# mschauer/ZigZagBoomerang.jl

Hardware: AMD Instinct MI355X
Metric: reflection events/sec, d=16384 local ZigZag (spdmp), ensemble of independent chains (higher is better)
Workload: dtype f64

## Files before the change

zigzagboomerang.jl_amd/csrc/pdmp_engine.hpp:

```cpp
#pragma once
#include <cstdint>
#include <string>
#include <vector>

#include "../../include/pdmp_mi355.h"
#ifdef PDMP_EXTRA_KERNELS
#include "../../include/pdmp_debug.h"
#endif

namespace pdmp {

struct alignas(64) ZzRec {
    double x;
    double th;
    double t;
    double I;
    double t_old;
    double a, b;
    uint64_t acc;
};
static_assert(sizeof(ZzRec) == 64, "record must be one 64-byte sector");

struct alignas(128) TrRec {
    double x, th, tx, I;
    double g, gd, tg;
    uint64_t acc;
    double a, b, t_old, tprop;
    double gb, gdb, tacc, pad;
};
static_assert(sizeof(TrRec) == 128, "tracked record must be one 128-byte line");
struct alignas(128) TrRecP {
    double x, th, tx, I;
    double g, gd, tg;
    uint64_t acc;
    double c, c100, gam0, gam1;
    double gam2, gam3, tacc, gam4;
};
static_assert(sizeof(TrRecP) == 128 && offsetof(TrRecP, tacc) == offsetof(TrRec, tacc), "same line, same tacc slot");

struct alignas(128) TrLine {
    double key0, told0, key1, told1;
    double th0, g0, gd0, tg0;
    double th1, g1, gd1, tg1;
    double c0, c100_0, c1, c100_1;
};
static_assert(sizeof(TrLine) == 128, "one line per coordinate pair");
struct alignas(32) TrCold {
    double x, tx, I;
    uint64_t acc;
};
static_assert(sizeof(TrCold) == 32, "one sector per coordinate");

struct alignas(128) DevChain {
    pdmp_chain_counters c;
    uint64_t seed;
    double t0;
    double t_event;
    double tl_scale;
    uint64_t pad[3];
};
static_assert(sizeof(DevChain) == 128, "chain header is 128 bytes");

#if defined(__HIPCC__)
__device__ __forceinline__ DevChain devchain_fresh(uint64_t seed, double t0, uint64_t ntrace, uint64_t nevents, uint64_t ndraw_main) {
    DevChain h;
    h.c.t_last = t0;
    h.c.num = 0;
    h.c.nacc = 0;
    h.c.nrefresh = 0;
    h.c.ntrace = ntrace;
    h.c.nevents = nevents;
    h.c.ndraw_main = ndraw_main;
    h.c.ndraw_global = 0;
    h.c.status = PDMP_CHAIN_OK;
    h.c.reserved = 0;
    h.seed = seed;
    h.t0 = t0;
    h.t_event = t0;
    h.tl_scale = 0.0;
    for (int k = 0; k < 3; ++k) h.pad[k] = 0;
    return h;
}

constexpr uint32_t PDMP_PRIO_TURN = 256u;
struct PrioTurn {
    uint32_t slot, it;
    __device__ __forceinline__ PrioTurn() : slot((uint32_t)__builtin_amdgcn_s_getreg(4 | (0 << 6) | (3 << 11)) & 3u), it(0) {}
    __device__ __forceinline__ void step() {
        if ((it & (PDMP_PRIO_TURN - 1u)) == 0u) {
            const uint32_t pr = ((it / PDMP_PRIO_TURN) + slot) & 3u;
            switch (pr) {
                case 0: __builtin_amdgcn_s_setprio(0); break;
                case 1: __builtin_amdgcn_s_setprio(1); break;
                case 2: __builtin_amdgcn_s_setprio(2); break;
                default: __builtin_amdgcn_s_setprio(3); break;
            }
        }
        it += 1;
    }
};

#ifndef PDMP_PRIO_LAG_K
#define PDMP_PRIO_LAG_K 32u
#endif
constexpr uint32_t PDMP_PRIO_BOARD_ROWS = 1u << 15, PDMP_PRIO_BOARD_SLOTS = 16u;
constexpr uint32_t PDMP_PRIO_BOARD_WORDS = PDMP_PRIO_BOARD_ROWS * PDMP_PRIO_BOARD_SLOTS;
struct PrioLag {
    PrioTurn turn;
    uint32_t* row;
    uint32_t slot, tag, it;
    double t_begin, scale;
    __device__ __forceinline__ PrioLag(uint32_t* board, uint32_t epoch, double t_begin_, double T) : row(nullptr), slot(0), tag(epoch << 24), it(0), t_begin(t_begin_), scale(0.0) {
        const double span = T - t_begin_;
        if (board != nullptr && epoch != 0u && span > 0.0 && span < __builtin_inf()) {
            const uint32_t xcc = (uint32_t)__builtin_amdgcn_s_getreg(20 | (0 << 6) | (3 << 11));
            const uint32_t hw = (uint32_t)__builtin_amdgcn_s_getreg(4 | (4 << 6) | (11 << 11));
            slot = (uint32_t)__builtin_amdgcn_s_getreg(4 | (0 << 6) | (3 << 11)) & (PDMP_PRIO_BOARD_SLOTS - 1u);
            row = board + (size_t)(((xcc << 12) | hw) & (PDMP_PRIO_BOARD_ROWS - 1u)) * PDMP_PRIO_BOARD_SLOTS;
            scale = 16777216.0 / span;
        }
    }
    __device__ __forceinline__ void step(double t_last, int lane) {
        if (row == nullptr) {
            turn.step();
            return;
        }
        if ((it & (PDMP_PRIO_LAG_K - 1u)) == 0u) {
            const double f = (t_last - t_begin) * scale;
            const uint32_t q = (f > 0.0) ? ((f < 16777214.0) ? (uint32_t)f : 0xfffffeu) : 0u;
            if (lane == 0) __hip_atomic_store(row + slot, tag | q, __ATOMIC_RELAXED, __HIP_MEMORY_SCOPE_AGENT);
            uint32_t w = 0u;
            if (lane < (int)PDMP_PRIO_BOARD_SLOTS) w = __hip_atomic_load(row + lane, __ATOMIC_RELAXED, __HIP_MEMORY_SCOPE_AGENT);
            const uint32_t wq = w & 0xffffffu;
            const bool behind = lane < (int)PDMP_PRIO_BOARD_SLOTS && (w & 0xff000000u) == tag && wq != 0xffffffu && (wq < q || (wq == q && (uint32_t)lane < slot));
            const uint32_t rank = (uint32_t)__popcll(__ballot(behind));
            switch (rank) {
                case 0: __builtin_amdgcn_s_setprio(3); break;
                case 1: __builtin_amdgcn_s_setprio(2); break;
                case 2: __builtin_amdgcn_s_setprio(1); break;
                default: __builtin_amdgcn_s_setprio(0); break;
            }
        }
        it += 1;
    }
    __device__ __forceinline__ void finish(int lane) {
        if (row != nullptr && lane == 0) __hip_atomic_store(row + slot, tag | 0xffffffu, __ATOMIC_RELAXED, __HIP_MEMORY_SCOPE_AGENT);
    }
};
#endif

struct CoordConst {
    double c, c100;
    uint32_t cp, k;
    double gam[5];
};
static_assert(sizeof(CoordConst) == 64, "half a line");

struct BarrierEntry {
    double lo, hi;
    double klo, khi;
    uint32_t rules;
    uint32_t pad;
};
static_assert(sizeof(BarrierEntry) == 40, "barrier table entry");
constexpr uint64_t BARRIER_ACT_HIT = 0, BARRIER_ACT_REFLECT = 1, BARRIER_ACT_UNFREEZE = 2;

struct ZzTables {
    const uint32_t* __restrict__ colptr;
    const uint32_t* __restrict__ rowval;
    const double* __restrict__ bval;
    const double* __restrict__ tval;
    const double* __restrict__ gmu_b;
    const double* __restrict__ gmu_t;
    const uint32_t* __restrict__ sptr;
    const uint32_t* __restrict__ sidx;
    const uint32_t* __restrict__ qptr;
    const uint8_t* __restrict__ pos;
    const uint8_t* __restrict__ selfpos;
    const double* __restrict__ c_shared;
    const double2* __restrict__ c2_shared;
    const CoordConst* __restrict__ cc_shared;
    const double* __restrict__ sigma;
    const double* __restrict__ gam8;
    const uint16_t* __restrict__ nb16;
};

constexpr uint32_t PDMP_LAUNCH_COUNT_LIMIT = 0xC0000000u;

struct ZzRunParams {
    ZzTables tb;
    ZzRec* rec;
    double* keys;
    DevChain* hdr;
    pdmp_event* ev;
    double* c_chain;
    double* dbg;
    int64_t dbg_cap;
    const uint64_t* __restrict__ blob;
    const uint32_t* __restrict__ tix;
    uint32_t blob_w, blob_w_pad, blob_sw, blob_pw, blob_kmax;
    uint32_t common_tix;
    int64_t d;
    int64_t dk;
    int64_t trace_cap;
    uint32_t nblk;
    uint32_t nblk_pad;
    double T;
    double factor;
    double lambda_ref;
    int32_t flags;
    int32_t adapt;
    int32_t has_refresh;
    int32_t move_all;
    int32_t force_spec4;
    int32_t track_two_sums;
    int32_t track_mean;
    uint32_t count_limit;
    uint32_t typ_extra;
    double hw_gain, hw_ahead;
    uint32_t hw_target;
    int32_t n_cu;
    int32_t helper_wave;
    uint32_t* prio_board;
    uint32_t prio_epoch;
    void* tl_lines;
    void* tl_cold;
    int32_t lattice_n;
    uint32_t lattice_magic;
    const uint64_t* __restrict__ g8_line;
// ... 368 lines not shown
```

zigzagboomerang.jl_amd/csrc/pdmp_trackp.hip:

```cpp
#include <hip/hip_runtime.h>

#include <cstdint>

#include "../../include/pdmp_detmath.h"
#include "pdmp_device.hpp"
#include "pdmp_engine.hpp"

namespace pdmp {

namespace {

__device__ __forceinline__ uint32_t w_grp8_min_u32(uint32_t v) {
    uint32_t o = (uint32_t)__builtin_amdgcn_mov_dpp((int)v, 0xB1, 0xf, 0xf, true);
    v = (o < v) ? o : v;
    o = (uint32_t)__builtin_amdgcn_mov_dpp((int)v, 0x4E, 0xf, 0xf, true);
    v = (o < v) ? o : v;
    o = (uint32_t)__builtin_amdgcn_mov_dpp((int)v, 0x141, 0xf, 0xf, true);
    return (o < v) ? o : v;
}
__device__ __forceinline__ uint32_t p_enc(double key, double tb, uint32_t pos) {
    double dlt = key - tb;
    dlt = (dlt > 0.0) ? dlt : 0.0;
    const uint32_t b = __float_as_uint((float)dlt);
    return (((b >= 8u) ? b - 8u : 0u) & ~7u) | pos;
}
__device__ __forceinline__ uint32_t p_thr(double tau, double tb) {
    double dlt = tau - tb;
    dlt = (dlt > 0.0) ? dlt : 0.0;
    return __float_as_uint((float)dlt) + 1u;
}
__device__ __forceinline__ double p_dec(uint32_t bits, double tb) {
    return pdmp_below(tb + (double)__uint_as_float(bits & ~7u));
}
constexpr uint32_t P_INFBITS = 0x7f7ffff8u;
__device__ __forceinline__ uint32_t lbf_pos(const unsigned char* smem, uint32_t b) {
    return reinterpret_cast<const uint32_t*>(smem)[b] & 7u;
}

}

template <bool HW, bool BIG = false>
struct WL {
    static_assert(!(HW && BIG), "the two-wave form keeps 2048 block bounds");
    static constexpr uint32_t NBLK = BIG ? 8192 : 2048;
    static constexpr uint32_t XO = (NBLK - 2048) * 4;
    static constexpr uint32_t LB = 0;
    static constexpr uint32_t EX = XO + 8192;
    static constexpr uint32_t URING = XO + 8704;
    static constexpr uint32_t SLB = XO + (HW ? 9792 : 9728);
    static constexpr uint32_t TB = XO + (HW ? 9920 : 9856);
    static constexpr uint32_t ACL = XO + (HW ? 10048 : 9984);
    static constexpr uint32_t NB = XO + (HW ? 10144 : 10016);
    static constexpr uint32_t CTL = 10272;
    static constexpr uint32_t HPF = 10336;
    static constexpr uint32_t RING = 10464;
    static constexpr int CMAX = HW ? 64 : 56;
    static constexpr uint32_t WIN = HW ? 256u : 128u;
    static constexpr uint32_t BYTES = HW ? RING + 512 * 16 : NB + 128;
};
constexpr uint32_t W_NR = 512;
constexpr uint32_t W_BYTES_1W = WL<false>::BYTES, W_BYTES_BIG = WL<false, true>::BYTES;
constexpr uint32_t W_BYTES_HW = WL<true>::BYTES;
constexpr int W_AMAX = 8;
#ifndef W_GROW
#define W_GROW 1.02
#define W_SHRINK 0.98
#define W_SLACK 5u
#endif
#ifndef W_HEAD_ONE_PASS
#define W_HEAD_ONE_PASS 1
#endif
#define W_TARGET_HW 48u
#define W_GAIN_HW 0.3
#define W_TARGET_1W 44u
#define W_TARGET_1W_MAX_PER_CU 12
#define W_NHYP 8
#define W_NHYP_1W 4
#define W_PF_AHEAD 1.0
static_assert(WL<false>::BYTES <= 10240, "16 chains per CU: 160 KB / 16");
static_assert(WL<false>::URING + WL<false>::WIN * 8 <= WL<false>::SLB && WL<false, true>::URING + WL<false, true>::WIN * 8 <= WL<false, true>::SLB &&
                  WL<false>::ACL + W_AMAX * 2 <= WL<false>::NB,
              "the one-wave forms' ring of draws ends where the event blocks begin");
static_assert(WL<false, true>::BYTES <= 40960, "d <= 65536: 4 chains per CU (one per SIMD), 160 KB / 4");
static_assert(W_BYTES_HW == WL<true>::RING + W_NR * 16 && W_BYTES_HW <= 20480, "8 chains per CU: 160 KB / 8");
struct WCtl {
    uint32_t filled;
    uint32_t consumed;
    uint32_t exitf;
    uint32_t pad;
    double pf_tau, pf_dt, pf_tb;
};
typedef volatile __attribute__((address_space(3))) WCtl* WCtlPtr;
__device__ __forceinline__ WCtlPtr w_ctl(unsigned char* smem, uint32_t offset) {
    return (WCtlPtr)(__attribute__((address_space(3))) unsigned char*)(smem + offset);
}

namespace {
__device__ __forceinline__ bool nb_has(const uint4 nb, uint32_t v2) {
    const uint32_t x0 = nb.x ^ v2, x1 = nb.y ^ v2, x2 = nb.z ^ v2, x3 = nb.w ^ v2;
    const uint32_t z = ((x0 - 0x00010001u) & ~x0) | ((x1 - 0x00010001u) & ~x1) | ((x2 - 0x00010001u) & ~x2) | ((x3 - 0x00010001u) & ~x3);
    return (z & 0x80008000u) != 0u;
}
__device__ __forceinline__ uint32_t nb_count(const uint4 nb) {
    const uint64_t hi = ((uint64_t)nb.w << 32) | nb.z, lo = ((uint64_t)nb.y << 32) | nb.x;
    const uint32_t ph = (~hi == 0ull) ? 4u : ((uint32_t)__builtin_clzll(~hi) >> 4);
    const uint32_t pl = (~lo == 0ull) ? 4u : ((uint32_t)__builtin_clzll(~lo) >> 4);
    return 8u - ((ph == 4u) ? 4u + pl : ph);
}
}

template <bool LAT>
__device__ __forceinline__ void trackp_helper(const ZzRunParams& P, unsigned char* smem, const int lane, const int64_t chain, const uint64_t seed,
                                           const uint64_t nm0) {
    using L = WL<true, false>;
    const WCtlPtr ctl = w_ctl(smem, L::CTL);
    double2* const ring = reinterpret_cast<double2*>(smem + L::RING);
    const uint4* const lb4 = reinterpret_cast<const uint4*>(smem + L::LB);
    const int64_t d = P.d;
    const char* const recb = reinterpret_cast<const char*>(reinterpret_cast<const TrRecP*>(P.rec) + chain * d);
    const char* const kpb = reinterpret_cast<const char*>(reinterpret_cast<const double2*>(P.keys) + chain * P.dk);
    uint16_t* const HPF = reinterpret_cast<uint16_t*>(smem + L::HPF);
    uint32_t filled = 0, sink = 0;
    double pf_done = -PDMP_INF;
    for (;;) {
        if (ctl->exitf != 0u) break;
        bool did = false;
        const uint32_t cons = ctl->consumed;
        while (filled + 64u <= cons + W_NR) {
            const uint32_t n = filled + (uint32_t)lane;
            const double u = pdmp_u01(seed, PDMP_STREAM_MAIN, nm0 + (uint64_t)n);
            ring[n & (W_NR - 1u)] = make_double2(u, pdmp_log(u));
            PDMP_LDS_ORDER();
            filled += 64u;
            if (lane == 0) ctl->filled = filled;
            did = true;
        }
        const double tau = ctl->pf_tau, dts = ctl->pf_dt, tbs = ctl->pf_tb;
        const double target = tau + P.hw_ahead * dts;
        if (target > pf_done) {
            const uint32_t lo = (pf_done > tbs) ? p_thr(pf_done, tbs) : 0u;
            const uint32_t hi0 = p_thr(target, tbs), hi = (hi0 < P_INFBITS) ? hi0 : P_INFBITS - 1u;
            uint32_t cm = 0;
#pragma unroll
            for (int j = 7; j >= 0; --j) {
                const uint4 v = lb4[lane + 64 * j];
                cm = (cm << 4) | ((v.x > lo && v.x <= hi) ? 1u : 0u) | ((v.y > lo && v.y <= hi) ? 2u : 0u) | ((v.z > lo && v.z <= hi) ? 4u : 0u) |
                     ((v.w > lo && v.w <= hi) ? 8u : 0u);
            }
            const uint32_t ncl = (uint32_t)__builtin_popcount(cm);
            const uint32_t incl = scan_add_u32(ncl);
            const uint32_t tot = (uint32_t)__builtin_amdgcn_readlane((int)incl, 63);
            uint32_t ix = incl - ncl, m_ = cm;
            while (m_ != 0u) {
                const uint32_t j = (uint32_t)(__ffs((int)m_) - 1);
// ... 98 lines not shown
                const uint32_t k = 8u * (uint32_t)s + (uint32_t)j;
                const bool in = 8u * k + (uint32_t)g < nblk;
                const double v = kp[(in ? (size_t)64 * k : (size_t)0) + (size_t)lane].x;
                vn[j] = in ? v : PDMP_INF;
            }
        };
        load8(0);
#pragma unroll
        for (int s = 0; s < 32; ++s) {
            double vc[8];
#pragma unroll
            for (int j = 0; j < 8; ++j) vc[j] = vn[j];
            __builtin_amdgcn_sched_barrier(0);
            if (s + 1 < 32) load8(s + 1);
            __builtin_amdgcn_sched_barrier(0);
            double keep = PDMP_INF;
            uint32_t kpos = 0u;
#pragma unroll
            for (int j = 0; j < 8; ++j) {
                const double v = vc[j];
                const double m = grp8_min_f64(v);
                const uint32_t pos = w_grp8_min_u32((v == m) ? (uint32_t)gl : 8u);
                keep = (gl == j) ? m : keep;
                kpos = (gl == j) ? pos : kpos;
            }
            asm volatile("" : "+v"(keep), "+v"(kpos));
            bm[s] = keep;
            bpos[s >> 3] |= (kpos & 7u) << (4 * (s & 7));
            asm volatile("" : "+v"(bpos[s >> 3]));
            mloc = min_f64(mloc, keep);
        }
        tb = wave_min_f64(mloc);
#pragma unroll
        for (int s = 0; s < 32; ++s)
            lbf[64 * s + 8 * gl + g] = (bm[s] < PDMP_INF) ? p_enc(bm[s], tb, (bpos[s >> 3] >> (4 * (s & 7))) & 7u) : P_INFBITS;
    } else {
        double mloc = t_last;
        for (uint32_t b = lane; b < nblk; b += 64) {
            const double2* p = kp + (size_t)b * 8;
#pragma unroll
            for (int q = 0; q < 8; ++q) mloc = min_f64(mloc, p[q].x);
        }
        tb = wave_min_f64(mloc);
        for (uint32_t b = lane; b < W_NBLK; b += 64) {
            uint32_t e = P_INFBITS;
            if (b < nblk) {
                const double2* p = kp + (size_t)b * 8;
                double mk = p[0].x;
                uint32_t mi = 0;
#pragma unroll
                for (int q = 1; q < 8; ++q) {
                    const double v = p[q].x;
                    if (v < mk) {
                        mk = v;
                        mi = q;
                    }
                }
                e = (mk < PDMP_INF) ? p_enc(mk, tb, mi) : P_INFBITS;
            }
            lbf[b] = e;
        }
    }
    PDMP_LDS_ORDER();

    uint64_t ph[10] = {0, 0, 0, 0, 0, 0, 0, 0, 0, 0};
    uint64_t ph_t0 = PROF ? (uint64_t)__builtin_readcyclecounter() : 0;
    uint64_t ph_rounds = 0, ph_guess = 0;
    uint64_t ph_iters = 0, ph_raw = 0, ph_zone = 0, ph_eval = 0;
#ifdef PDMP_PHASE_MARKS
#define WMARK(k) asm volatile("; WPHASE " #k)
#else
#define WMARK(k)
#endif
#define WPHASE(k)                                                         \
    do {                                                                  \
        WMARK(k);                                                         \
        if (PROF) {                                                       \
            const uint64_t now_ = (uint64_t)__builtin_readcyclecounter(); \
            ph[k] += now_ - ph_t0;                                        \
            ph_t0 = now_;                                                 \
        }                                                                 \
    } while (0)

    PrioLag prio((!HW && !BIG) ? P.prio_board : nullptr, P.prio_epoch, t_last, T);
    bool need_rebase = false;
    uint32_t idle = 0;
    bool running = stop_before || (t_event < T);
    while (running) {
        prio.step(t_last, lane);
        if (dnacc >= trace_room) {
            status = PDMP_CHAIN_TRACE_FULL;
            break;
        }
        if (dnm >= P.count_limit) {
            status = PDMP_CHAIN_PAUSED;
            break;
        }
        if (HW) {
            if (lane == 0) ctl->consumed = dnm;
            while (ctl->filled < dnm + W_WIN) __builtin_amdgcn_s_sleep(1);
            PDMP_LDS_ORDER();
        } else {
            const uint32_t ulim = dnm + W_WIN;
            while (ufilled < ulim) {
                const uint32_t n = ufilled + (uint32_t)lane;
                if (!uhave) {
                    unext = pdmp_u01(seed, PDMP_STREAM_MAIN, nm0 + (uint64_t)n);
                    uhave = true;
                }
                const uint32_t uend = (ufilled + 64u < ulim) ? ufilled + 64u : ulim;
                if (n >= uflushed && n < uend) uring[n & (W_WIN - 1u)] = unext;
                uflushed = uend;
                if (uend != ufilled + 64u) break;
                ufilled += 64u;
                uhave = false;
            }
            PDMP_LDS_ORDER();
        }
        WPHASE(7);
        auto draw = [&](uint32_t n) -> double {
            if (HW) return ring[n & (W_NR - 1u)].x;
            return uring[n & (W_WIN - 1u)];
        };
        auto drawlog = [&](uint32_t n) -> double {
            if (HW) return ring[n & (W_NR - 1u)].y;
            return pdmp_log(draw(n));
        };
        int C = 0;
        bool stalled = false, finished = false;
        double dt_used = 0.0;
        uint32_t Cc = 0;
        double tau = 0.0, mql_sel = 0.0;
        bool tau_clipped = false;
        {
            uint32_t kk[32];
            auto loadc = [&](int c) {
#pragma unroll
                for (int j = 0; j < 8; ++j) {
                    const uint4 v = reinterpret_cast<const uint4*>(lbf)[512 * c + lane + 64 * j];
                    kk[4 * j + 0] = v.x;
                    kk[4 * j + 1] = v.y;
                    kk[4 * j + 2] = v.z;
                    kk[4 * j + 3] = v.w;
                }
            };
            auto lanemin = [&]() -> uint32_t {
                uint32_t m_ = kk[0];
#pragma unroll
                for (int j = 1; j < 32; ++j) m_ = (kk[j] < m_) ? kk[j] : m_;
                return m_;
            };
            uint32_t mloc = 0xffffffffu;
#pragma unroll
            for (int c = 0; c < NCH; ++c) {
                loadc(c);
                const uint32_t m_ = lanemin();
                mloc = (m_ < mloc) ? m_ : mloc;
            }
            uint32_t mqb = wave_min_u32_dpp(mloc);
            double mql = p_dec(mqb, tb);
            if (mqb < P_INFBITS && (need_rebase || mql - tb > 0.25)) {
                mloc = 0xffffffffu;
#pragma unroll
                for (int c = 0; c < NCH; ++c) {
                    if (NCH > 1) loadc(c);
#pragma unroll
                    for (int j = 0; j < 32; ++j)
                        kk[j] = (kk[j] >= P_INFBITS) ? P_INFBITS : p_enc(p_dec(kk[j], tb), mql, kk[j] & 7u);
#pragma unroll
                    for (int j = 0; j < 8; ++j)
                        reinterpret_cast<uint4*>(lbf)[512 * c + lane + 64 * j] = make_uint4(kk[4 * j + 0], kk[4 * j + 1], kk[4 * j + 2], kk[4 * j + 3]);
                    const uint32_t m_ = lanemin();
// ... 163 lines not shown
#pragma unroll
                for (uint32_t q = 0; q < 8; ++q) rank += (km[q] < own) ? 1u : 0u;
            }
            PDMP_LDS_ORDER();
            rsum = (uint32_t)__builtin_amdgcn_readlane((int)scan_add_u32(isev ? rank : 0u), 63);
        }
        bool slot = isev;
        if (rsum != (uint32_t)(nev * (nev - 1) / 2)) {
            const double mn = wave_min_f64(own);
            const uint32_t bsel = wave_min_u32_dpp((isev && own == mn) ? cblk : 0xffffffffu);
            slot = isev && cblk == bsel;
            nev = 1;
        }
        {
            const bool wrongpos = isev && (c_pb & 7u) != cpos;
            const uint32_t wr = wave_min_u32_dpp(wrongpos ? rank : 0xffffffffu);
            if (wr < (uint32_t)nev) nev = (int)wr;
        }
        const uint32_t pdst = ((slot && rank < (uint32_t)nev) ? rank : 63u) << 2;
        auto push32 = [&](uint32_t v) -> uint32_t { return (uint32_t)__builtin_amdgcn_ds_permute((int)pdst, (int)v); };
        auto push64 = [&](double v) -> double {
            const int lo = __builtin_amdgcn_ds_permute((int)pdst, __double2loint(v)), hi = __builtin_amdgcn_ds_permute((int)pdst, __double2hiint(v));
            return __hiloint2double(hi, lo);
        };
        const double e_km = push64(c_km), e_rs = push64(c_rs), e_tp = push64(c_tp);
        const double e_th = push64(c_th), e_g = push64(c_g), e_gd = push64(c_gd), e_tg = push64(c_tg), e_c = push64(c_c2.x), e_c100 = push64(c_c2.y);
        double e_gmu = 0.0;
        if (tmean) e_gmu = push64(c_gmu);
        const uint32_t e_bu = push32(cblk | (c_pb << 16));
        uint4 e_nb = make_uint4(~0u, ~0u, ~0u, ~0u);
        if (!LAT) e_nb = make_uint4(push32(c_nb.x), push32(c_nb.y), push32(c_nb.z), push32(c_nb.w));
        PDMP_LDS_ORDER();
        WPHASE(9);
        C = nev;
        if (PROF) ph_iters += 1;
        if (PROF) ph_raw += (uint64_t)Cc;
        const int Craw = (int)Cc;
        asm volatile("" ::"v"(c_th), "v"(c_g), "v"(c_gd), "v"(c_tg), "v"(c_c2.x), "v"(c_c2.y), "v"(c_nb.x), "v"(c_gmu));
        if (C == 0) {
            if (tau_clipped && !crowded && __ballot(isc && c_km <= tau) == 0) break;
            if (++idle > 4096u) {
                status = PDMP_CHAIN_STALLED;
                break;
            }
            seldt = uniform_f64(dt_used * 2.0);
            continue;
        }
        bool ev = lane < C;
        const double tp = ev ? e_km : PDMP_INF;
        const double rest = ev ? e_rs : PDMP_INF;
        const double tprop_i = ev ? e_tp : 0.0;
        const uint32_t blk = e_bu & 0xffffu, pbe = e_bu >> 16;
        const double th = e_th, g_i = e_g, gd_i = e_gd, tg_i = e_tg;
        const double2 c_i2 = make_double2(e_c, e_c100);
        const uint4 nb_i = LAT ? make_uint4(~0u, ~0u, ~0u, ~0u) : e_nb;
        const uint32_t i = ev ? (blk * 8u + (pbe & 7u)) : 0u;
        const uint32_t rarg = blk * 8u + (pbe >> 4);
        const double c_i = c_i2.x;
        PDMP_LDS_ORDER();
        if (ev) SLB[lane] = (uint16_t)blk;
        PDMP_LDS_ORDER();
        WPHASE(0);
        uint32_t rc_i = 0xffffu, k_i;
        if (LAT) {
            const uint32_t col_i = __umulhi(i, nmagic);
            const uint32_t row_i = i - col_i * nlat;
            rc_i = ev ? (row_i | (col_i << 8)) : 0xffffu;
            k_i = 1u + (col_i > 0u ? 1u : 0u) + (row_i > 0u ? 1u : 0u) + (row_i + 1u < nlat ? 1u : 0u) + (col_i + 1u < nlat ? 1u : 0u);
        } else {
            k_i = nb_count(nb_i);
        }
        PDMP_LDS_ORDER();
        const double g_now = g_i + gd_i * (tp - tg_i);
        const double gmu_i = e_gmu;
        const double l = pos_part(((tmean == 2) ? g_now - gmu_i : g_now) * th);
        const double told_i = tprop_i;
        const double g_told = g_i + gd_i * (told_i - tg_i);
        const double a_i = c_i + (tmean ? g_told - gmu_i : g_told) * th;
        const double b_i = c_i2.y + th * gd_i;
        const double lbound = pos_part(a_i + b_i * (tp - told_i));
        const uint32_t ex_i = k_i - 1u;
        uint32_t off = 2u * (uint32_t)lane;
        bool acc = false;
        {
            const uint32_t etyp = P.typ_extra;
            const uint64_t pl1 = __ballot(ev && (ex_i & 1u)), pl2 = __ballot(ev && (ex_i & 2u)), pl4 = __ballot(ev && (ex_i & 4u));
            auto offsets = [&](uint64_t ab) -> uint32_t {
                const uint64_t a1 = ab & pl1, a2 = ab & pl2, a4 = ab & pl4;
                const uint32_t n1 = __builtin_amdgcn_mbcnt_hi((uint32_t)(a1 >> 32), __builtin_amdgcn_mbcnt_lo((uint32_t)a1, 0u));
                const uint32_t n2 = __builtin_amdgcn_mbcnt_hi((uint32_t)(a2 >> 32), __builtin_amdgcn_mbcnt_lo((uint32_t)a2, 0u));
                const uint32_t n4 = __builtin_amdgcn_mbcnt_hi((uint32_t)(a4 >> 32), __builtin_amdgcn_mbcnt_lo((uint32_t)a4, 0u));
                return 2u * (uint32_t)lane + n1 + 2u * n2 + 4u * n4;
            };
            uint64_t accb = 0;
            const uint64_t tg0_ = PROF ? (uint64_t)__builtin_readcyclecounter() : 0;
            constexpr int NHYP = HW ? W_NHYP : W_NHYP_1W;
            if (NHYP > 0) {
                uint64_t hb[NHYP > 0 ? NHYP : 1];
                double uj[NHYP > 0 ? NHYP : 1];
#pragma unroll
                for (int j = 0; j < NHYP; ++j) {
                    const uint32_t oj = off + etyp * (uint32_t)j;
                    uj[j] = draw(dnm + ((oj < W_WIN - 1u) ? oj : W_WIN - 1u));
                }
#pragma unroll
                for (int j = 0; j < NHYP; ++j) {
                    const uint32_t oj = off + etyp * (uint32_t)j;
                    hb[j] = __ballot((int)ev & (int)(oj + 1u + k_i <= W_WIN) & (int)(uj[j] * lbound < l));
                }
                const uint64_t odd = __ballot(ev && ex_i != etyp);
                uint64_t live = ~0ull;
#pragma unroll
                for (int j = 0; j < NHYP; ++j) {
                    const uint64_t rem = hb[j] & live;
                    const uint64_t low = rem & (0ull - rem);
                    accb |= low;
                    live = (low & ~odd) ? ~(low | (low - 1ull)) : 0ull;
                }
                if (accb != 0ull) off = offsets(accb);
            }
            if (PROF) ph_guess += (uint64_t)__builtin_readcyclecounter() - tg0_;
            for (int round = 0; round < 72; ++round) {
                if (PROF) ph_rounds += 1;
                const bool inwin = ev && (off + 1u + k_i <= W_WIN);
                const double u = draw(dnm + ((off < W_WIN - 1u) ? off : W_WIN - 1u));
                acc = inwin && (u * lbound < l);
                const uint64_t nb_ = __ballot(acc);
                if (nb_ == accb) break;
                accb = nb_;
                off = offsets(accb);
            }
        }
        const uint32_t cost = ev ? (acc ? (1u + k_i) : 2u) : 0u;
        {
            const uint64_t outb = __ballot(ev && !(off + 1u + k_i <= W_WIN));
            if (outb) {
                const int cut = __ffsll((unsigned long long)outb) - 1;
                C = (cut < C) ? cut : C;
            }
        }
        WPHASE(1);
        {
            uint64_t ab = __ballot(acc) & ((C < 64) ? ((1ull << C) - 1ull) : ~0ull);
            if (__popcll(ab) > AMAXT) {
                uint64_t m_ = ab;
                for (int q = 0; q < AMAXT; ++q) m_ &= m_ - 1;
                C = __ffsll((unsigned long long)m_) - 1;
            }
        }
        uint32_t rekey_by = 0xffffffffu;
        if (LAT && HW) {
            uint32_t* const ZA = reinterpret_cast<uint32_t*>(smem + L::NB);
            const uint64_t ab = __ballot(acc) & ((C < 64) ? ((1ull << C) - 1ull) : ~0ull);
            if (lane < W_AMAX) ZA[lane] = 0x00fffefeu;
            PDMP_LDS_ORDER();
            if (acc && lane < C)
                ZA[__builtin_amdgcn_mbcnt_hi((uint32_t)(ab >> 32), __builtin_amdgcn_mbcnt_lo((uint32_t)ab, 0u))] = rc_i | ((uint32_t)lane << 16);
            PDMP_LDS_ORDER();
            const uint4 z0 = reinterpret_cast<const uint4*>(ZA)[0], z1 = reinterpret_cast<const uint4*>(ZA)[1];
            const uint32_t zz[8] = {z0.x, z0.y, z0.z, z0.w, z1.x, z1.y, z1.z, z1.w};
            bool conf = false;
#pragma unroll
            for (int q = 0; q < W_AMAX; ++q) {
                const uint32_t m = zz[q] >> 16;
                const uint32_t sad = __builtin_amdgcn_sad_u8(rc_i, zz[q] & 0xffffu, 0u);
                conf = conf || (((uint32_t)lane > m) && (sad <= 1u || (sad <= 2u && acc)));
                if (sad <= 1u && (uint32_t)lane < m && m < rekey_by) rekey_by = m;
            }
            const uint64_t cb = __ballot(conf) & ((C < 64) ? ((1ull << C) - 1ull) : ~0ull);
            if (cb) {
                const int c0 = __ffsll((unsigned long long)cb) - 1;
                C = (c0 < C) ? c0 : C;
            }
        } else if (LAT) {
            uint64_t confb = 0;
            uint64_t ab = __ballot(acc) & ((C < 64) ? ((1ull << C) - 1ull) : ~0ull);
            while (ab) {
                const int m = __ffsll((unsigned long long)ab) - 1;
                ab &= ab - 1;
                const uint32_t rcm = (uint32_t)__builtin_amdgcn_readlane((int)rc_i, m);
                const uint32_t sad = __builtin_amdgcn_sad_u8(rc_i, rcm, 0u);
                const uint64_t hit = __ballot(sad <= 1u || (sad <= 2u && acc));
                confb |= hit & (~0ull << (m + 1));
                if (sad <= 1u && lane < m && (uint32_t)m < rekey_by) rekey_by = (uint32_t)m;
            }
            const uint64_t cb = confb & ((C < 64) ? ((1ull << C) - 1ull) : ~0ull);
            if (cb) {
                const int c0 = __ffsll((unsigned long long)cb) - 1;
                C = (c0 < C) ? c0 : C;
            }
        } else {
            const uint64_t ab0 = __ballot(acc) & ((C < 64) ? ((1ull << C) - 1ull) : ~0ull);
            const int nacc0 = __popcll(ab0);
            if (acc && lane < C) {
                const int sl = __popcll(ab0 & ((1ull << lane) - 1ull));
                NB4[sl] = nb_i;
                ACL[sl] = (uint16_t)lane;
            }
            PDMP_LDS_ORDER();
            const uint32_t jt = (g < nacc0) ? (uint32_t)NB16[lane] : 0xffffu;
            const uint32_t jt2 = jt | (jt << 16), i2 = i | (i << 16);
            uint64_t confb = 0, ghit = 0;
            uint64_t ab = ab0;
            for (int sl = 0; sl < nacc0; ++sl) {
                const int m = __ffsll((unsigned long long)ab) - 1;
                ab &= ab - 1;
                const uint4 nbm = NB4[sl];
                const bool d1 = ev && nb_has(nbm, i2);
                confb |= __ballot(d1) & (~0ull << (m + 1));
                if (d1 && lane < m && (uint32_t)m < rekey_by) rekey_by = (uint32_t)m;
                ghit |= __ballot(g > sl && jt != 0xffffu && nb_has(nbm, jt2));
            }
            if (ghit) {
                const int gs = (__ffsll((unsigned long long)ghit) - 1) >> 3;
                const int r2 = (int)ACL[gs];
                confb |= 1ull << r2;
            }
            const uint64_t cb = confb & ((C < 64) ? ((1ull << C) - 1ull) : ~0ull);
            if (cb) {
                const int c0 = __ffsll((unsigned long long)cb) - 1;
                C = (c0 < C) ? c0 : C;
            }
        }
        if (PROF) ph_zone += (uint64_t)C;
        const bool violated0 = acc && (l >= lbound);
        int vsel = -1;
        uint64_t vb_adapt = 0;
        {
            const uint64_t vb = __ballot(violated0) & ((C < 64) ? ((1ull << C) - 1ull) : ~0ull);
            if (vb) {
// ... 4 lines not shown
                    C = vsel;
                }
            }
        }
        ev = lane < C;
        acc = acc && ev;
        if (PROF) ph_eval += (uint64_t)C;
        const uint64_t accball = __ballot(acc);
        const int nacc_it = __popcll(accball);
        if (LAT && !HW && acc) ACL[__popcll(accball & ((1ull << lane) - 1ull))] = (uint16_t)lane;
        PDMP_LDS_ORDER();
        WPHASE(2);
        struct GOut {
            bool gact, mem, selfl, adapted;
            double c_new, c100_new;
            uint32_t ea, ia, blka, jm, cand_a;
            double tpa, gj, gdj, keyj, xa, txa, Ia, th_ia, rowmin_a;
            uint64_t acc_ia;
        };
        double key2 = PDMP_INF;
        auto group_stage = [&](const int base, const int ng, const bool first) -> GOut {
            GOut o;
            const int g0 = 8 - ng;
            const bool gact = g >= g0;
            uint32_t ea = 0u;
            if (HW) {
                uint64_t m_ = accball;
                const int want = base + g - g0;
#pragma unroll
                for (int n = 0; n < AMAXT; ++n) {
                    const uint32_t pos = m_ ? (uint32_t)(__ffsll((unsigned long long)m_) - 1) : 0u;
                    m_ &= m_ - 1ull;
                    ea = (want == n) ? pos : ea;
                }
            } else {
                ea = gact ? (uint32_t)ACL[g - g0] : 0u;
            }
            const uint32_t ia_b = (uint32_t)__builtin_amdgcn_ds_bpermute((int)(ea << 2), (int)i);
            const uint32_t off_b = (uint32_t)__builtin_amdgcn_ds_bpermute((int)(ea << 2), (int)off);
            const uint32_t ia = gact ? ia_b : 0u;
            const uint32_t blka = gact ? (uint32_t)SLB[ea] : 0u;
            const double tpa_b = bperm_f64(tp, ea);
            const double tpa = gact ? tpa_b : 0.0;
            const uint32_t offa = gact ? off_b : 0u;
            uint32_t ka = 0, jm = ia;
            bool mem = false;
            if (LAT) {
                const uint32_t cola = __umulhi(ia, nmagic), rowa = ia - cola * nlat;
                const bool hasL = cola > 0u, hasU = rowa > 0u, hasD = rowa + 1u < nlat, hasR = cola + 1u < nlat;
                ka = gact ? (1u + (hasL ? 1u : 0u) + (hasU ? 1u : 0u) + (hasD ? 1u : 0u) + (hasR ? 1u : 0u)) : 0u;
                mem = gact && (uint32_t)gl < ka;
                const uint32_t pos = (uint32_t)gl;
                const uint32_t cand5[5] = {ia - nlat, ia - 1u, ia, ia + 1u, ia + nlat};
                const bool has5[5] = {hasL, hasU, true, hasD, hasR};
                uint32_t seen = 0;
#pragma unroll
                for (int q = 0; q < 5; ++q) {
                    if (has5[q]) {
                        if (seen == pos && mem) jm = cand5[q];
                        seen += 1;
                    }
                }
            } else {
                const uint32_t jraw = gact ? (uint32_t)NB16[8 * (g - g0) + gl] : 0xffffu;
                mem = jraw != 0xffffu;
                jm = mem ? jraw : ia;
            }
            TrRecP* const rj = rec + jm;
            TrRecP* const ria = rec + ia;
            double gam = 0.0;
            if (LAT) {
                if (mem) gam = (gl == 0) ? ria->gam0 : (gl == 1) ? ria->gam1 : (gl == 2) ? ria->gam2 : (gl == 3) ? ria->gam3 : ria->gam4;
            } else {
                if (mem) gam = P.tb.gam8[(size_t)ia * 8 + (size_t)gl];
            }
            const double th_ia = ria->th;
            double xa = ria->x, txa = ria->tx, Ia = ria->I;
            const uint64_t acc_ia = ria->acc;
            const double thj0 = rj->th, gj0 = rj->g, gdj0 = rj->gd, tgj = rj->tg;
            double gmu_j = 0.0;
            if (tmean) gmu_j = rj->tacc;
            double2 cjm2 = *reinterpret_cast<const double2*>(&rj->c);
            asm volatile("" : "+v"(cjm2.x), "+v"(cjm2.y));
            const double resta_b = bperm_f64(rest, ea);
            const uint32_t rarga_b = (uint32_t)__builtin_amdgcn_ds_bpermute((int)(ea << 2), (int)rarg);
            const bool selfl = mem && jm == ia;
            const bool adapted = selfl && ((vb_adapt >> ea) & 1ull) != 0ull;
            if (adapted) {
                cjm2.x = cjm2.x * P.factor;
                cjm2.y = cjm2.x / 100;
            }
            const double thj = selfl ? -th_ia : thj0;
            const double gj = gj0 + gdj0 * (tpa - tgj);
            const double gdj = gdj0 + gam * (-2.0 * th_ia);
            double a2l, b2l, key2l;
            {
                const bool mine = gact || !first;
                const uint32_t dix = mine ? (offa + 1u + (uint32_t)gl) : (off + 1u);
                const double Lg = drawlog(dnm + ((dix < W_WIN - 1u) ? dix : W_WIN - 1u));
                const double cc = mine ? cjm2.x : c_i, cc100 = mine ? cjm2.y : c_i2.y;
                const double gg0 = mine ? gj : g_now, tt = mine ? thj : th, gdd = mine ? gdj : gd_i;
                const double gg = tmean ? gg0 - (mine ? gmu_j : gmu_i) : gg0;
                a2l = cc + gg * tt;
                b2l = cc100 + tt * gdd;
                key2l = (mine ? tpa : tp) + poisson_time_L(a2l, b2l, Lg);
            }
            const double keyj = mem ? key2l : PDMP_INF;
            if (first) {
                if (__ballot(ev && !acc && gact) != 0) {
                    const double Le = drawlog(dnm + ((off + 1u < W_WIN - 1u) ? off + 1u : W_WIN - 1u));
                    const double a2e = c_i + (tmean ? g_now - gmu_i : g_now) * th;
                    const double b2e = c_i2.y + th * gd_i;
                    const double k2e = tp + poisson_time_L(a2e, b2e, Le);
                    if (gact) key2l = k2e;
                }
                key2 = key2l;
            }
            if (selfl) {
                const double dtx = tpa - txa;
                const double xn = xa + th_ia * dtx;
                Ia = Ia + dtx * ((xa + xn) * 0.5);
                xa = xn;
                txa = tpa;
            }
            const double kin = (mem && (jm >> 3) == blka) ? keyj : PDMP_INF;
            const double kinmin = grp8_min_f64(kin);
            const uint32_t wkey = (gact && kin == kinmin) ? (((uint32_t)gl << 3) | (jm & 7u)) : 0xffu;
            const uint32_t jwin = w_grp8_min_u32(wkey);
            const bool restwins = resta_b <= kinmin;
            const double rowmin_a = restwins ? resta_b : kinmin;
            const uint32_t cand_a = restwins ? (rarga_b & 7u) : (jwin & 7u);
            const double keymin = grp8_min_f64(keyj);
            if (gact && gl == 0) EX[ea] = min_f64(rowmin_a, keymin);
            asm volatile("" ::"v"(xa), "v"(txa), "v"(Ia), "v"(acc_ia));
            o.gact = gact;
            o.mem = mem;
            o.selfl = selfl;
            o.adapted = adapted;
            o.c_new = cjm2.x;
            o.c100_new = cjm2.y;
            o.ea = ea;
            o.ia = ia;
            o.blka = blka;
            o.jm = jm;
            o.cand_a = cand_a;
            o.tpa = tpa;
            o.gj = gj;
            o.gdj = gdj;
            o.keyj = keyj;
            o.xa = xa;
            o.txa = txa;
            o.Ia = Ia;
            o.th_ia = th_ia;
            o.rowmin_a = rowmin_a;
            o.acc_ia = acc_ia;
            return o;
        };
        const GOut G0 = group_stage(0, nacc_it, true);
        double rowmin = PDMP_INF;
        uint32_t cand = i;
        if (ev && !acc) {
            const bool mine = key2 < rest || (key2 == rest && i < rarg);
            rowmin = mine ? key2 : rest;
            cand = mine ? i : rarg;
        }
        if (ev && !acc) EX[lane] = rowmin;
// ... 29 lines not shown
            seldt = uniform_f64(dt_used * (((int)Rc >= Craw) ? W_GROW : (((int)Rc + (int)W_SLACK < Craw) ? W_SHRINK : 1.0)));
        }
        WPHASE(4);
        const bool commit = ev && (uint32_t)lane < Rc;
        if (commit && !acc) {
            if (!(rekey_by < Rc)) kp[i] = make_double2(key2, tp);
            lbf[blk] = (rowmin < PDMP_INF) ? p_enc(rowmin, tb, cand & 7u) : P_INFBITS;
        }
        const uint64_t acc_c = accball & ((Rc < 64u) ? ((1ull << Rc) - 1ull) : ~0ull);
        auto commit_groups = [&](const GOut& o) {
            const bool gcommit = o.gact && o.ea < Rc;
            if (gcommit) {
                TrRecP* const rj = rec + o.jm;
                TrRecP* const ria = rec + o.ia;
                if (o.mem) {
                    rj->g = o.gj;
                    rj->gd = o.gdj;
                    rj->tg = o.tpa;
                    kp[o.jm] = make_double2(o.keyj, o.tpa);
                }
                if (o.selfl) {
                    ria->x = o.xa;
                    ria->th = -o.th_ia;
                    ria->tx = o.txa;
                    ria->I = o.Ia;
                    ria->acc = o.acc_ia + 1;
                    if (o.adapted) *reinterpret_cast<double2*>(&ria->c) = make_double2(o.c_new, o.c100_new);
                    if (evout) {
                        const uint32_t rnk = (uint32_t)__popcll(acc_c & ((1ull << o.ea) - 1ull));
                        pdmp_event e;
                        e.t = o.tpa;
                        e.i = (int64_t)o.ia;
                        e.x = o.xa;
                        e.theta = -o.th_ia;
                        evout[ntrace0 + dnacc + rnk] = e;
                    }
                }
                if (gl == 0) lbf[o.blka] = (o.rowmin_a < PDMP_INF) ? p_enc(o.rowmin_a, tb, o.cand_a) : P_INFBITS;
            }
            return gcommit;
        };
        const bool gc0 = commit_groups(G0);
        PDMP_LDS_ORDER();
        WPHASE(5);
        {
            if (gc0 && G0.mem && (G0.jm >> 3) != G0.blka && G0.keyj < PDMP_INF) atomicMin(&lbf[G0.jm >> 3], p_enc(G0.keyj, tb, G0.jm & 7u));
        }
        PDMP_LDS_ORDER();
        WPHASE(6);
        if (Rc > 0u) {
            const uint32_t costL = (uint32_t)__builtin_amdgcn_readlane((int)cost, (int)(Rc - 1u));
            const uint32_t offL = (uint32_t)__builtin_amdgcn_readlane((int)off, (int)(Rc - 1u));
            dnum += Rc;
            idle = 0;
            dnacc += (uint32_t)__popcll(acc_c);
            dnm += offL + costL;
            t_last = readlane_f64(tp, (int)(Rc - 1u));
            if (acc_c) t_event = readlane_f64(tp, 63 - __builtin_clzll(acc_c));
        }
        if (vsel >= 0) {
            const double tpv = readlane_f64(tp, vsel);
            const uint32_t iv = (uint32_t)__builtin_amdgcn_readlane((int)i, vsel);
            if (lane == 0) kp[iv].y = tpv;
            dnum += 1;
            vnacc = 1;
            dnm += 1;
            t_last = tpv;
            status = PDMP_CHAIN_BOUND_VIOLATED;
        }
        if (status != PDMP_CHAIN_OK) break;
        PDMP_LDS_ORDER();
    }

    if (PROF && P.dbg && chain == 0 && lane == 0) {
        for (int q = 0; q < 10; ++q) P.dbg[q] = (double)ph[q];
        P.dbg[10] = (double)ph_iters;
        P.dbg[11] = (double)ph_raw;
        P.dbg[12] = (double)ph_zone;
        P.dbg[13] = (double)ph_eval;
        P.dbg[14] = (double)ph_rounds;
        P.dbg[15] = (double)ph_guess;
    }
#undef WPHASE
    prio.finish(lane);
    if (HW && lane == 0) ctl->exitf = 1u;
    if (lane == 0) {
        hdr->c.t_last = t_last;
        hdr->t_event = t_event;
        hdr->c.num += dnum;
        hdr->c.nacc += dnacc + vnacc;
        hdr->c.ntrace = ntrace0 + dnacc;
        hdr->c.nevents += dnacc;
        hdr->c.ndraw_main = nm0 + dnm;
        hdr->c.status = status;
    }
}

template <bool PROF, bool LAT>
__global__ __launch_bounds__(64) __attribute__((amdgpu_waves_per_eu(4, 4))) void zz_local_trackp_kernel(ZzRunParams P) {
    trackp_body<PROF, LAT, false, false>(P);
}
template <bool PROF>
__global__ __launch_bounds__(64) __attribute__((amdgpu_waves_per_eu(1, 2))) void zz_local_trackp_big_kernel(ZzRunParams P) {
    trackp_body<PROF, true, false, true>(P);
}
template <bool PROF, bool LAT>
__global__ __launch_bounds__(128) __attribute__((amdgpu_waves_per_eu(4, 4))) void zz_local_trackp2_kernel(ZzRunParams P) {
    trackp_body<PROF, LAT, true, false>(P);
}

bool zz_trackp_supported(const ZzRunParams& p) {
    const bool lattice = p.lattice_n >= 16 && p.lattice_n <= 256 && p.d <= (int64_t)WL<false, true>::NBLK * 8;
    const bool graph = p.lattice_n == 0 && p.tb.nb16 != nullptr && p.tb.gam8 != nullptr && p.d <= (int64_t)WL<false>::NBLK * 8;
    return (lattice || graph) && p.tb.gmu_t == nullptr && !p.track_two_sums && !p.has_refresh && p.d >= 2048;
}

bool zz_trackp_big(int64_t d) { return d > (int64_t)WL<false>::NBLK * 8; }

int launch_zz_local_trackp(const ZzRunParams& p, int64_t nchains, void* stream, const char** kname) {
    dim3 grid((unsigned)nchains), block(64);
    ZzRunParams q = p;
    q.nblk = (uint32_t)((p.d + 7) / 8);
    const bool lat = p.lattice_n != 0;
    if (kname) *kname = zz_trackp_big(p.d) ? "zz_local_trackp_big_kernel" : p.helper_wave ? (lat ? "zz_local_trackp2_kernel" : "zz_local_trackp2_kernel<LAT=false>")
                                                                                        : (lat ? "zz_local_trackp_kernel" : "zz_local_trackp_kernel<LAT=false>");
    if (!p.helper_wave && !(q.hw_gain > 0.0)) {
        if (nchains <= (int64_t)W_TARGET_1W_MAX_PER_CU * (p.n_cu > 0 ? p.n_cu : 256) || zz_trackp_big(p.d)) {
            q.hw_gain = W_GAIN_HW;
            q.hw_target = W_TARGET_1W;
        } else {
            q.hw_target = 0u;
        }
    }
    if (zz_trackp_big(p.d)) {
        if (p.dbg) hipLaunchKernelGGL((zz_local_trackp_big_kernel<true>), grid, block, W_BYTES_BIG, (hipStream_t)stream, q);
        else hipLaunchKernelGGL((zz_local_trackp_big_kernel<false>), grid, block, W_BYTES_BIG, (hipStream_t)stream, q);
        return (int)hipGetLastError();
    }
    if (p.helper_wave) {
        dim3 block2(128);
        if (!(q.hw_gain > 0.0)) {
            q.hw_gain = W_GAIN_HW;
            q.hw_target = W_TARGET_HW;
            q.hw_ahead = W_PF_AHEAD;
        }
        if (lat) {
            if (p.dbg) hipLaunchKernelGGL((zz_local_trackp2_kernel<true, true>), grid, block2, W_BYTES_HW, (hipStream_t)stream, q);
            else hipLaunchKernelGGL((zz_local_trackp2_kernel<false, true>), grid, block2, W_BYTES_HW, (hipStream_t)stream, q);
        } else {
            if (p.dbg) hipLaunchKernelGGL((zz_local_trackp2_kernel<true, false>), grid, block2, W_BYTES_HW, (hipStream_t)stream, q);
            else hipLaunchKernelGGL((zz_local_trackp2_kernel<false, false>), grid, block2, W_BYTES_HW, (hipStream_t)stream, q);
        }
        return (int)hipGetLastError();
    }
    if (lat) {
        if (p.dbg) hipLaunchKernelGGL((zz_local_trackp_kernel<true, true>), grid, block, W_BYTES_1W, (hipStream_t)stream, q);
        else hipLaunchKernelGGL((zz_local_trackp_kernel<false, true>), grid, block, W_BYTES_1W, (hipStream_t)stream, q);
    } else {
        if (p.dbg) hipLaunchKernelGGL((zz_local_trackp_kernel<true, false>), grid, block, W_BYTES_1W, (hipStream_t)stream, q);
        else hipLaunchKernelGGL((zz_local_trackp_kernel<false, false>), grid, block, W_BYTES_1W, (hipStream_t)stream, q);
    }
    return (int)hipGetLastError();
}

__global__ __launch_bounds__(256) void zz_trackp_consts_kernel(TrRecP* __restrict__ rec, const CoordConst* __restrict__ cc,
                                                              const uint16_t* __restrict__ nb16, const double* __restrict__ gmu, int64_t d, int64_t nchains) {
    const int64_t i = (int64_t)blockIdx.x * 256 + threadIdx.x;
// ... 64 lines not shown
```

Before: 1.450 billion.

## Re-derive priority-board state on demand and add optional early member prefetch

PrioLag no longer keeps its row pointer, slot, tag, start time and scale in registers for the whole loop. It re-derives them every K iterations from kernel params and an atomic load of the header's t_last, which is meant to lower register pressure in the hot loop. A new W_EARLY_MEMBERS option (off by default) issues early loads of neighbour record words so their latency overlaps the later gather. The cost is extra getreg, load and arithmetic work at each board step. Re-reading t_begin from the header also assumes hdr->c.t_last is unchanged until the end of the kernel.

```diff
diff --git a/zigzagboomerang.jl_amd/csrc/pdmp_engine.hpp b/zigzagboomerang.jl_amd/csrc/pdmp_engine.hpp
--- a/zigzagboomerang.jl_amd/csrc/pdmp_engine.hpp
+++ b/zigzagboomerang.jl_amd/csrc/pdmp_engine.hpp
@@ -106,45 +106,70 @@
 constexpr uint32_t PDMP_PRIO_BOARD_ROWS = 1u << 15, PDMP_PRIO_BOARD_SLOTS = 16u;
 constexpr uint32_t PDMP_PRIO_BOARD_WORDS = PDMP_PRIO_BOARD_ROWS * PDMP_PRIO_BOARD_SLOTS;
 struct PrioLag {
-    PrioTurn turn;
-    uint32_t* row;
-    uint32_t slot, tag, it;
-    double t_begin, scale;
-    __device__ __forceinline__ PrioLag(uint32_t* board, uint32_t epoch, double t_begin_, double T) : row(nullptr), slot(0), tag(epoch << 24), it(0), t_begin(t_begin_), scale(0.0) {
-        const double span = T - t_begin_;
-        if (board != nullptr && epoch != 0u && span > 0.0 && span < __builtin_inf()) {
-            const uint32_t xcc = (uint32_t)__builtin_amdgcn_s_getreg(20 | (0 << 6) | (3 << 11));
-            const uint32_t hw = (uint32_t)__builtin_amdgcn_s_getreg(4 | (4 << 6) | (11 << 11));
-            slot = (uint32_t)__builtin_amdgcn_s_getreg(4 | (0 << 6) | (3 << 11)) & (PDMP_PRIO_BOARD_SLOTS - 1u);
-            row = board + (size_t)(((xcc << 12) | hw) & (PDMP_PRIO_BOARD_ROWS - 1u)) * PDMP_PRIO_BOARD_SLOTS;
-            scale = 16777216.0 / span;
+    uint32_t it;
+    struct Row {
+        uint32_t* row;
+        uint32_t slot, tag;
+        double t_begin, scale;
+    };
+    __device__ __forceinline__ PrioLag() : it(0) {}
+    static __device__ __forceinline__ uint32_t wave_slot() { return (uint32_t)__builtin_amdgcn_s_getreg(4 | (0 << 6) | (3 << 11)); }
+    static __device__ __forceinline__ Row derive(uint32_t* board, uint32_t epoch, const double* t_begin_p, double T) {
+        Row r;
+        r.row = nullptr;
+        r.slot = 0u;
+        r.tag = epoch << 24;
+        r.t_begin = 0.0;
+        r.scale = 0.0;
+        if (board != nullptr && epoch != 0u) {
+            r.t_begin = __longlong_as_double((long long)__hip_atomic_load(reinterpret_cast<const uint64_t*>(t_begin_p), __ATOMIC_RELAXED, __HIP_MEMORY_SCOPE_WAVEFRONT));
+            const double span = T - r.t_begin;
+            if (span > 0.0 && span < __builtin_inf()) {
+                const uint32_t xcc = (uint32_t)__builtin_amdgcn_s_getreg(20 | (0 << 6) | (3 << 11));
+                const uint32_t hw = (uint32_t)__builtin_amdgcn_s_getreg(4 | (4 << 6) | (11 << 11));
+                r.slot = wave_slot() & (PDMP_PRIO_BOARD_SLOTS - 1u);
+                r.row = board + (size_t)(((xcc << 12) | hw) & (PDMP_PRIO_BOARD_ROWS - 1u)) * PDMP_PRIO_BOARD_SLOTS;
+                r.scale = 16777216.0 / span;
+            }
         }
+        return r;
     }
-    __device__ __forceinline__ void step(double t_last, int lane) {
-        if (row == nullptr) {
-            turn.step();
-            return;
-        }
+    __device__ __forceinline__ void step(uint32_t* board, uint32_t epoch, const double* t_begin_p, double T, double t_last, int lane) {
+        static_assert(PDMP_PRIO_TURN % PDMP_PRIO_LAG_K == 0u, "the turns' cadence is a multiple of the board's");
         if ((it & (PDMP_PRIO_LAG_K - 1u)) == 0u) {
-            const double f = (t_last - t_begin) * scale;
-            const uint32_t q = (f > 0.0) ? ((f < 16777214.0) ? (uint32_t)f : 0xfffffeu) : 0u;
-            if (lane == 0) __hip_atomic_store(row + slot, tag | q, __ATOMIC_RELAXED, __HIP_MEMORY_SCOPE_AGENT);
-            uint32_t w = 0u;
-            if (lane < (int)PDMP_PRIO_BOARD_SLOTS) w = __hip_atomic_load(row + lane, __ATOMIC_RELAXED, __HIP_MEMORY_SCOPE_AGENT);
-            const uint32_t wq = w & 0xffffffu;
-            const bool behind = lane < (int)PDMP_PRIO_BOARD_SLOTS && (w & 0xff000000u) == tag && wq != 0xffffffu && (wq < q || (wq == q && (uint32_t)lane < slot));
-            const uint32_t rank = (uint32_t)__popcll(__ballot(behind));
-            switch (rank) {
-                case 0: __builtin_amdgcn_s_setprio(3); break;
-                case 1: __builtin_amdgcn_s_setprio(2); break;
-                case 2: __builtin_amdgcn_s_setprio(1); break;
-                default: __builtin_amdgcn_s_setprio(0); break;
+            const Row r = derive(board, epoch, t_begin_p, T);
+            if (r.row == nullptr) {
+                if ((it & (PDMP_PRIO_TURN - 1u)) == 0u) {
+                    const uint32_t pr = ((it / PDMP_PRIO_TURN) + (wave_slot() & 3u)) & 3u;
+                    switch (pr) {
+                        case 0: __builtin_amdgcn_s_setprio(0); break;
+                        case 1: __builtin_amdgcn_s_setprio(1); break;
+                        case 2: __builtin_amdgcn_s_setprio(2); break;
+                        default: __builtin_amdgcn_s_setprio(3); break;
+                    }
+                }
+            } else {
+                const double f = (t_last - r.t_begin) * r.scale;
+                const uint32_t q = (f > 0.0) ? ((f < 16777214.0) ? (uint32_t)f : 0xfffffeu) : 0u;
+                if (lane == 0) __hip_atomic_store(r.row + r.slot, r.tag | q, __ATOMIC_RELAXED, __HIP_MEMORY_SCOPE_AGENT);
+                uint32_t w = 0u;
+                if (lane < (int)PDMP_PRIO_BOARD_SLOTS) w = __hip_atomic_load(r.row + lane, __ATOMIC_RELAXED, __HIP_MEMORY_SCOPE_AGENT);
+                const uint32_t wq = w & 0xffffffu;
+                const bool behind = lane < (int)PDMP_PRIO_BOARD_SLOTS && (w & 0xff000000u) == r.tag && wq != 0xffffffu && (wq < q || (wq == q && (uint32_t)lane < r.slot));
+                const uint32_t rank = (uint32_t)__popcll(__ballot(behind));
+                switch (rank) {
+                    case 0: __builtin_amdgcn_s_setprio(3); break;
+                    case 1: __builtin_amdgcn_s_setprio(2); break;
+                    case 2: __builtin_amdgcn_s_setprio(1); break;
+                    default: __builtin_amdgcn_s_setprio(0); break;
+                }
             }
         }
         it += 1;
     }
-    __device__ __forceinline__ void finish(int lane) {
-        if (row != nullptr && lane == 0) __hip_atomic_store(row + slot, tag | 0xffffffu, __ATOMIC_RELAXED, __HIP_MEMORY_SCOPE_AGENT);
+    __device__ __forceinline__ void finish(uint32_t* board, uint32_t epoch, const double* t_begin_p, double T, int lane) {
+        const Row r = derive(board, epoch, t_begin_p, T);
+        if (r.row != nullptr && lane == 0) __hip_atomic_store(r.row + r.slot, r.tag | 0xffffffu, __ATOMIC_RELAXED, __HIP_MEMORY_SCOPE_AGENT);
     }
 };
 #endif
diff --git a/zigzagboomerang.jl_amd/csrc/pdmp_trackp.hip b/zigzagboomerang.jl_amd/csrc/pdmp_trackp.hip
--- a/zigzagboomerang.jl_amd/csrc/pdmp_trackp.hip
+++ b/zigzagboomerang.jl_amd/csrc/pdmp_trackp.hip
@@ -70,6 +70,9 @@
 #ifndef W_HEAD_ONE_PASS
 #define W_HEAD_ONE_PASS 1
 #endif
+#ifndef W_EARLY_MEMBERS
+#define W_EARLY_MEMBERS 0
+#endif
 #define W_TARGET_HW 48u
 #define W_GAIN_HW 0.3
 #define W_TARGET_1W 44u
@@ -334,12 +337,13 @@
         }                                                                 \
     } while (0)
 
-    PrioLag prio((!HW && !BIG) ? P.prio_board : nullptr, P.prio_epoch, t_last, T);
+    PrioLag prio;
+    uint32_t* const prio_board = (!HW && !BIG) ? P.prio_board : nullptr;
     bool need_rebase = false;
     uint32_t idle = 0;
     bool running = stop_before || (t_event < T);
     while (running) {
-        prio.step(t_last, lane);
+        prio.step(prio_board, P.prio_epoch, &hdr->c.t_last, P.T, t_last, lane);
         if (dnacc >= trace_room) {
             status = PDMP_CHAIN_TRACE_FULL;
             break;
@@ -669,6 +673,43 @@
         const uint32_t ex_i = k_i - 1u;
         uint32_t off = 2u * (uint32_t)lane;
         bool acc = false;
+        constexpr int EARLY = (!HW && !BIG) ? W_EARLY_MEMBERS : 0;
+        uint32_t early_w0 = 0u, early_w1 = 0u;
+        uint64_t early_done = 0ull;
+        auto early_members = [&](const uint64_t ab) -> uint32_t {
+            const bool mine = ((ab >> lane) & 1ull) != 0ull;
+            const uint32_t s = __builtin_amdgcn_mbcnt_hi((uint32_t)(ab >> 32), __builtin_amdgcn_mbcnt_lo((uint32_t)ab, 0u));
+            const bool send = mine && s < (uint32_t)W_AMAX;
+            uint32_t jn = 0u;
+            bool ask = false;
+            if (LAT) {
+                const uint32_t got = (uint32_t)__builtin_amdgcn_ds_permute((int)((send ? 4u * s : 63u) << 2), (int)(send ? i + 1u : 0u));
+                const uint32_t v = (uint32_t)__builtin_amdgcn_mov_dpp((int)got, 0x00, 0xf, 0xf, true);
+                const uint32_t ia = v - 1u;
+                const uint32_t cola = __umulhi(ia, nmagic), rowa = ia - cola * nlat;
+                uint32_t q = (uint32_t)lane & 3u;
+                asm volatile("" : "+v"(q));
+                const bool horiz = ((q + 1u) & 2u) == 0u, up = q >= 2u;
+                const uint32_t coord = horiz ? cola : rowa, step = horiz ? nlat : 1u;
+                const uint32_t room = up ? nlat - 1u - coord : coord;
+                jn = up ? ia + step : ia - step;
+                ask = ((int)(v != 0u) & (int)(room != 0u) & (int)(jn < (uint32_t)d)) != 0;
+            } else {
+                uint32_t r = 0u;
+                const uint32_t nbw[4] = {nb_i.x, nb_i.y, nb_i.z, nb_i.w};
+#pragma unroll
+                for (uint32_t k = 0; k < 4u; ++k)
+                    r |= (uint32_t)__builtin_amdgcn_ds_permute((int)((send ? 8u * s + 2u * k : 63u) << 2), (int)(send ? ~nbw[k] : 0u));
+                const uint32_t wv = ~(uint32_t)__builtin_amdgcn_mov_dpp((int)r, 0xA0, 0xf, 0xf, true);
+                uint32_t sh = ((uint32_t)lane & 1u) << 4;
+                asm volatile("" : "+v"(sh));
+                jn = (wv >> sh) & 0xffffu;
+                ask = ((int)(jn != 0xffffu) & (int)(jn < (uint32_t)d)) != 0;
+            }
+            uint32_t w = 0u;
+            if (ask) w = *reinterpret_cast<const uint32_t*>(reinterpret_cast<const char*>(rec + jn) + 32);
+            return w;
+        };
         {
             const uint32_t etyp = P.typ_extra;
             const uint64_t pl1 = __ballot(ev && (ex_i & 1u)), pl2 = __ballot(ev && (ex_i & 2u)), pl4 = __ballot(ev && (ex_i & 4u));
@@ -705,6 +746,10 @@
                     live = (low & ~odd) ? ~(low | (low - 1ull)) : 0ull;
                 }
                 if (accb != 0ull) off = offsets(accb);
+                if (EARLY == 2) {
+                    early_done = accb;
+                    if (accb != 0ull) early_w0 = early_members(accb);
+                }
             }
             if (PROF) ph_guess += (uint64_t)__builtin_readcyclecounter() - tg0_;
             for (int round = 0; round < 72; ++round) {
@@ -733,6 +778,10 @@
                 uint64_t m_ = ab;
                 for (int q = 0; q < AMAXT; ++q) m_ &= m_ - 1;
                 C = __ffsll((unsigned long long)m_) - 1;
+            }
+            if (EARLY) {
+                const uint64_t rest = ab & ((C < 64) ? ((1ull << C) - 1ull) : ~0ull) & ~early_done;
+                if (rest != 0ull) early_w1 = early_members(rest);
             }
         }
         uint32_t rekey_by = 0xffffffffu;
@@ -903,6 +952,8 @@
             if (tmean) gmu_j = rj->tacc;
             double2 cjm2 = *reinterpret_cast<const double2*>(&rj->c);
             asm volatile("" : "+v"(cjm2.x), "+v"(cjm2.y));
+            if (EARLY == 2) asm volatile("" ::"v"(early_w0));
+            if (EARLY) asm volatile("" ::"v"(early_w1));
             const double resta_b = bperm_f64(rest, ea);
             const uint32_t rarga_b = (uint32_t)__builtin_amdgcn_ds_bpermute((int)(ea << 2), (int)rarg);
             const bool selfl = mem && jm == ia;
@@ -1098,7 +1149,7 @@
         P.dbg[15] = (double)ph_guess;
     }
 #undef WPHASE
-    prio.finish(lane);
+    prio.finish(prio_board, P.prio_epoch, &hdr->c.t_last, P.T, lane);
     if (HW && lane == 0) ctl->exitf = 1u;
     if (lane == 0) {
         hdr->c.t_last = t_last;
```

Result: no change. 1.461 billion (median of 4 runs) (+0.7%).
